# amazon-science/tubelet-transformer

Measured on AMD Instinct MI355X. Metric: clips/sec (TubeR CSN-152 AVA2.1 training step fwd+bwd+clip+AdamW, 32x256x340 clips; whole job), higher is better.
Workload: dtype bf16; 1 GPU; TubeR_CSN152_AVA21 train step, 2 clips/GPU of 3x32x256x340, dropout on, random-init name-hashed weights; global_batch=2, parallelism=dp1, launch_mode=hipgraph, lib_md5=41483701da62

## Files before the change

### include/tuber_hip.h

```cpp
#ifndef TUBER_HIP_H
#define TUBER_HIP_H

#ifdef __cplusplus
extern "C" {
#endif

typedef struct ihipStream_t* hipStream_t;

typedef struct TuberClipDesc {
    long long src_off;
    int H, W;
    int y1, x1, h, w;
    int flip, jitter;
    int hue, sat, val;
    int pad_;
} TuberClipDesc;

int tuber_attn_fwd(const void* Q, const long* mq, const void* K, const long* mk, const void* V, const long* mv, void* O, const long* mo, float* lse, const void* key_padding_mask, int B, int H, int Lq, int Lk, float scale, float pdrop, const void* seed_ptr, unsigned long long salt, hipStream_t stream);

int tuber_attn_bwd(const void* Q, const long* mq, const void* K, const long* mk, const void* V, const long* mv, const void* O, const long* mo, const float* lse, const void* key_padding_mask, const void* dO, const long* mdo, void* dQ, const long* mdq, void* dK, const long* mdk, void* dV, const long* mdv, float* delta, int B, int H, int Lq, int Lk, float scale, float pdrop, const void* seed_ptr, unsigned long long salt, hipStream_t stream);

int tuber_attn_wide_fwd(const void* q, const void* kv, void* o, int NQ, int HW, int T, float pdrop, const void* seed_ptr, unsigned long long salt, hipStream_t stream);

int tuber_attn_wide_bwd(const void* q, const void* kv, const void* dO, void* dq, void* dkv, int NQ, int HW, int T, float pdrop, const void* seed_ptr, unsigned long long salt, hipStream_t stream);

int tuber_blockout_conv1_supported(int c, int pn);

int tuber_blockout_conv1_fwd(const void* c4, const float* s4, const float* h4, const void* res, const float* rs, const float* rh, void* y, const void* w, long ldw, void* c1, float* st0, float* st1, long M, int pn, hipStream_t stream);

int tuber_blockout_conv1_fwd_mask(const void* c4, const float* s4, const float* h4, const void* res, const float* rs, const float* rh, void* y, void* ymask, const void* w, long ldw, void* c1, float* st0, float* st1, long M, int pn, hipStream_t stream);

int tuber_frames_resize(const void* src, void* tmp, void* dst, int nimg, int H, int W, int Ho, int Wo, const void* bounds_h, const void* kk_h, int ksize_h, const void* bounds_v, const void* kk_v, int ksize_v, int y0, int rows, hipStream_t stream);

int tuber_clip_prepare(const void* frames, const void* desc, const void* lut, const void* hsv_tab, void* out, void* mask, int N, int T, int Hmax, int Wmax, hipStream_t stream);

int tuber_clip_desc_bytes(void);

int tuber_comm_etimedout(void);

int tuber_comm_version(void);

const char* tuber_comm_last_error(void);

int tuber_comm_unique_id(void* id128);

int tuber_comm_init(const void* id128, int nranks, int rank, int device, void** comm_out);

int tuber_comm_init_timeout(const void* id128, int nranks, int rank, int device, int timeout_ms, void** comm_out);
// ... 273 lines not shown
```

### tubelet_transformer_amd/csrc/gen_header.py

```python
import glob
import os
import re

HERE = os.path.dirname(os.path.abspath(__file__))
ROOT = os.path.dirname(os.path.dirname(HERE))

DOC = {
    "tuber_gemm_nt_addproj": "packed attention in-projection with the positional embedding folded in: C = f(A).B^T + bias with f(A) = A + A2 for the output "
                             "columns [0, add_ncols) (q / k rows of in_proj_weight: with_pos_embed, models/transformer/transformer.py:150-159,215-240) and "
                             "f(A) = A for the v rows -- one GEMM instead of an add kernel and two GEMM launches. add_ncols % 128 == 0.",
    "tuber_bn_bwd_fa": "tuber_bn_bwd_finalize + tuber_bn_bwd_apply in ONE launch for short partial lists (layer3 / layer4 of the CSN body): every workgroup "
                       "derives the coefficients of its 128-channel strip from the R partial rows (fp64) and applies dx = cA*dz + cB*x + cC to its rows; "
                       "dgamma / dbeta accumulated by the first row chunk (NULL: frozen BatchNorm). autograd of nn.BatchNorm3d (ir_CSN_152.py:46,56,64,154).",
    "tuber_bn_bwd_fa_max_rows": "largest R tuber_bn_bwd_fa accepts.",
    "tuber_ln_bwd_dx": "tuber_layernorm_bwd (partial rows only) + the data-gradient tuber_gemm_nt of the linear layer in front of the LayerNorm in ONE launch: "
                       "autograd of tgt = norm(tgt + dropout(sublayer)) where the sublayer ends in out_proj / linear2 (models/transformer/transformer.py:160-167,229-247). "
                       "Every workgroup runs the LayerNorm backward of its 32 rows itself and multiplies the bf16 result from LDS with W on MFMA; the column-0 workgroups "
                       "store dx / dxd / the dgamma, dbeta partial rows ([tuber_ln_bwd_dx_blocks(M)][2E]) as the two-launch path does. dy2: a second gradient contribution (replaces "
                       "a tuber_axpby launch) or NULL; res: an existing gradient of the linear's input to add; cm / alpha: the ReLU / Dropout mask of that input.",
    "tuber_rows_dx2": "both data gradients of a packed attention in-projection with the positional embedding folded in (tuber_gemm_nt_addproj; "
                      "models/transformer/transformer.py:150-159,215-240) in ONE launch for few rows: dx = g.W over all N columns (+ res), dpos = g[:, :Nq].W[:Nq] "
                      "stored as a prefix of the same reduction. Replaces two tuber_gemm_nt launches per decoder in-projection.",
    "tuber_criterion_scale": "backward of tuber_criterion_loss's loss table in one launch: the stored per-layer gradients scaled by the incoming gradient of the [L][4] "
                             "losses (autograd of the weighted sum of loss terms, models/criterion.py:169-206 + train_tuber_ava.py loss weighting).",
# ... 210 lines not shown
    "tuber_block_out_bwd": "backward of the join: dz = dy*[y>0] and the partial statistics of bn4 (and of the down_sample BN).",
    "tuber_rowblock_count": "partial-stat rows written by the row-blocked reduce kernels for M rows.",
    "tuber_layernorm_fwd": "y = LayerNorm(Dropout_p(x) (+ res)) over E in {256, 2048}, eps 1e-5 (nn.LayerNorm, transformer.py:163-167,229-247,116-123; "
                           "transformer_layers.py:84,91,96,437-445); saves xhat (bf16) and rstd for backward.",
    "tuber_layernorm_bwd": "backward of tuber_layernorm_fwd: dx (gradient of res), dxd (gradient of x through the regenerated dropout mask) and dgamma/dbeta via block partials.",
    "tuber_layernorm_bwd_blocks": "blocks used by tuber_layernorm_bwd (partial = 2*blocks*E floats).",
    "tuber_reduce_rows": "out[c] (+)= sum_r P[r][c].",
    "tuber_colsum_blocks": "row blocks (size of `partial` / C) used by tuber_colsum.",
    "tuber_colsum": "bias gradient: out[c] (+)= sum_m g[m][c] for bf16 g.",
    "tuber_gemm_nt_set_cfg": "tuning hook: force tile configuration cfg for every later tuber_gemm_nt (-1 = automatic choice).",
    "tuber_stem_conv_fwd": "stem Conv3d(3,64,(3,7,7),s=(1,2,2),p=(1,3,3)) (ir_CSN_152.py:109-115) as an implicit MFMA GEMM from the fp32 NCDHW clip to NDHWC bf16, "
                           "with the partial statistics of the following BatchNorm; Wp = tuber_stem_pack_weight(conv1.weight).",
    "tuber_stem_conv_bwd_weight": "weight gradient of the stem conv ([64][441] fp32) as an implicit MFMA GEMM (no patch matrix in HBM).",
    "tuber_stem_conv_blocks": "persistent grid size of the stem conv forward = its partial-stat rows.",
    "tuber_stem_conv_wgrad_blocks": "workgroups (= [512][64] fp32 partial slabs) of tuber_stem_conv_bwd_weight.",
    "tuber_stem_pack_weight": "conv1.weight [64][441] fp32 -> [64][512] bf16 with k' = (c,kt,kh)*8 + kw (zero padded).",
    "tuber_stem_pool_fwd": "relu(bn1(.)) + MaxPool3d((1,3,3),s=(1,2,2),p=(0,1,1)) (ir_CSN_152.py:119-122) on NDHWC bf16, C=64; saves the argmax tap.",
    "tuber_stem_pool_bwd": "backward of the pool + relu(bn1(.)): dz and the BN-backward partial statistics.",
    "tuber_stem_pool_bwd_stat_rows": "partial-stat rows written by tuber_stem_pool_bwd.",
    "tuber_attn_fwd": "softmax(scale*QK^T + key_padding_mask)[dropout] V for 32-wide heads, operands read in place through strided token maps "
                      "{ld,sL,s1,s2,B2}: row(l,b) = l*sL + (b/B2)*s1 + (b%B2)*s2. Core of nn.MultiheadAttention "
                      "(transformer.py:159,227,237; tuber_ava.py:138; transformer_layers.py:81,88) and of the hand-rolled MHA (:156-167,306-366).",
    "tuber_attn_bwd": "gradients dQ, dK, dV of tuber_attn_fwd (P recomputed from the saved log-sum-exp).",
    "tuber_attn_wide_fwd": "single-query, 256-wide-head attention of the LSTR pooling decoder (TEMPORAL_DS_STRATEGY decode; "
                           "backbone_builder.py:74-78, transformer_layers.py:156-167,306-366): q [NQ,2048], kv [rows,4096]=[k|v], T<=8 slots per pixel.",
    "tuber_attn_wide_bwd": "gradients dq [NQ,2048] and dkv [rows,4096] of tuber_attn_wide_fwd.",
    "tuber_lsap": "rectangular linear sum assignment on HOST doubles; restates scipy.optimize.linear_sum_assignment (call sites "
                  "models/detr/matcher.py:80, matcher_ucf.py:82) incl. its tie-breaking.",
    "tuber_lsap_device": "the same assignment (scipy.optimize.linear_sum_assignment semantics incl. tie-breaking; matcher.py:80, matcher_ucf.py:82) for all "
                         "(decoder layer, clip) problems at once ON THE DEVICE, one thread per problem: match[l][b][t] = query of target t.",
    "tuber_grad_norm_clip_coef": "global L2 norm of the flat gradient buffer and the clip coefficient min(1, max_norm/(norm+1e-6)), left on the device: "
                                 "torch.nn.utils.clip_grad_norm_(model.parameters(), 0.1) (utils/video_action_recognition.py:153).  A non-finite norm "
                                 "yields coefficient -1 = skip the update and leaves the step count alone: the reference stops BEFORE optimizer.step() on a "
                                 "non-finite loss (video_action_recognition.py:195-198).",
    "tuber_adamw_segment": "AdamW update (torch.optim.AdamW semantics: decoupled decay, bias correction) of one contiguous flat segment with the "
                           "clip coefficient applied to the gradient on the fly (video_action_recognition.py:154; groups train_tuber_ava.py:41-58).",
    "tuber_grad_accum": "gradient accumulation over m micro-batches (DistributedDataParallel's mean over ranks reproduced on fewer GPUs: the mean of "
                        "independent per-rank backward passes, utils/model_utils.py:47-49) over a DEVICE table of nwin [begin, end) int64 windows of the flat "
                        "fp32 gradient buffer, in ONE launch: mode 0 acc = g, mode 1 acc += g, mode 2 g = (acc + g) * scale (scale_dev[0] when given). "
                        "Fixed order: sequential fp32 sum, then one multiply. g and acc 16-byte aligned.",
    "tuber_bn_stats_copy": "snapshot (restore = 0: arena <- buffers) or restore (restore = 1: buffers <- arena) of BatchNorm running statistics "
                           "(running_mean, running_var, num_batches_tracked of nn.BatchNorm3d, models/backbones/ir_CSN_152.py:46,56,64,154) in ONE launch over a "
                           "DEVICE table of nrows {address, arena offset in 32-bit words, words} int64 rows; max_words = the largest row.",
    "tuber_scale_f32": "x *= coef: gradient averaging after the RCCL all-reduce (DistributedDataParallel's mean, utils/model_utils.py:47-49).",
    "tuber_criterion_cost": "Hungarian matching cost C = w_bbox*L1 - w_giou*GIoU - w_class*p of every decoder layer at once, [L,B,Q,Tmax] fp32 "
                            "(HungarianMatcher.forward, models/detr/matcher.py:61-76 / matcher_ucf.py:61-78; generalized_box_iou utils/box_ops.py:41-65).",
# ... 101 lines not shown
```

### tubelet_transformer_amd/tape.py

```python
import numpy as np
import torch

from . import ab, lib

BF = torch.bfloat16


def _ceil(x, m):
    return (x + m - 1) // m * m


def _map(ld, sL, s1=0, s2=0, B2=1):
    return np.array([ld, sL, s1, s2, B2], dtype=np.int64)


class Tape:
    def __init__(self, store, train):
        self.store, self.train, self.dev = store, train, store.device
        self.ops = []
        self.g = {}
        self.alias = {}
        self.mask = {}
        self.premasked = set()
        self.stack = {}
# ... 407 lines not shown
            if acc == 2 and preq:
                if dbeta == dgamma + 4 * E:
                    st.defer.add(part, dgamma, 2 * E, 2 * E, nb, 1)
                else:
                    st.defer.add(part, dgamma, E, 2 * E, nb, 1)
                    st.defer.add(part + 4 * E, dbeta, E, 2 * E, nb, 1)
            return part, dgamma, dbeta, acc

        rec = _PendingLN(tp, g=g, gptr=gptr, ldg=ldg, g2=g2, xhat=xhat, rstd=rstd, gamma=gamma, dx=dx, dxd=dxd, p=p, salt=salt, M=M, E=E,
                         register=register)
        fusable = xreq and out is None and st.defer.enabled and not ab.on("no_ln_bwd_fusion") and id(tp.target(x)) in tp.lin_out
        chained = (xreq and out is not None and p == 0.0 and res is None and E == 256 and st.defer.enabled and not ab.on("no_ln_bwd_fusion")
                   and id(tp.target(x)) in tp.pair_ok and isinstance(tp.g.get(id(tp.target(x))), torch.Tensor))
        if not (fusable or chained):
            rec.force()
        if xreq:
            tp.put(x, dxd if p > 0.0 else dx)
        if rreq:
            tp.put(res, dx)
    tp.rec(bwd)
    return y


def attention(tp, roles, geom, kpm, pdrop, *tensors):
    st = tp.store
    B, H, Lq, Lk, qmap, kmap = geom
    (qi, qo), (ki, ko), (vi, vo) = roles
    tq, tk, tv = tensors[qi], tensors[ki], tensors[vi]
    dev = tq.device
    E = H * 32
    o = torch.empty(tq.shape[0], E, dtype=BF, device=dev)
    lse = torch.empty(B, H, Lq, dtype=torch.float32, device=dev)
    mq, mk, mv = _map(tq.shape[1], *qmap), _map(tk.shape[1], *kmap), _map(tv.shape[1], *kmap)
    mo = _map(E, *qmap)
    scale = 32 ** -0.5
    p = float(pdrop)
    salt = tp.salt()
    if tp.dry:
        tp.dry_log.append(("attention", dict(tensors=tensors, roles=roles, o=o, lse=lse, kpm=kpm, geom=geom, p=p, salt=salt)))
    else:
        lib.call("tuber_attn_fwd", tq.data_ptr() + 2 * qo, mq.ctypes.data, tk.data_ptr() + 2 * ko, mk.ctypes.data,
                 tv.data_ptr() + 2 * vo, mv.ctypes.data, o, mo.ctypes.data, lse, kpm, B, H, Lq, Lk, scale, float(p), st.seed, salt)
    if not tp.train:
        return o
    treq = [tp.needs(t) for t in tensors]
    if not any(treq):
        return o
    tp.mark(o)

    def bwd():
        g = tp.take(o)
        if g is None:
            return
        covered = [0] * len(tensors)
        for ti, _ in roles:
            covered[ti] += E
        grads = [torch.empty_like(t) if covered[i] >= t.shape[1] else torch.zeros_like(t) for i, t in enumerate(tensors)]
        delta = torch.empty(B, H, Lq, dtype=torch.float32, device=dev)
        lib.call("tuber_attn_bwd", tq.data_ptr() + 2 * qo, mq.ctypes.data, tk.data_ptr() + 2 * ko, mk.ctypes.data,
                 tv.data_ptr() + 2 * vo, mv.ctypes.data, o, mo.ctypes.data, lse, kpm, g, mo.ctypes.data,
                 grads[qi].data_ptr() + 2 * qo, mq.ctypes.data, grads[ki].data_ptr() + 2 * ko, mk.ctypes.data,
                 grads[vi].data_ptr() + 2 * vo, mv.ctypes.data, delta, B, H, Lq, Lk, scale, float(p), st.seed, salt)
        for t, gt, need in zip(tensors, grads, treq):
            if need:
                tp.put(t, gt)
    tp.rec(bwd)
    return o


def attention_wide(tp, q, kv, HW, T, pdrop):
    st = tp.store
    NQ = q.shape[0]
    o = torch.empty(NQ, 2048, dtype=BF, device=q.device)
    p = float(pdrop)
    salt = tp.salt()
    lib.call("tuber_attn_wide_fwd", q, kv, o, NQ, HW, T, float(p), st.seed, salt)
    if not tp.train:
        return o
    qreq, kreq = tp.needs(q), tp.needs(kv)
    if not (qreq or kreq):
        return o
    tp.mark(o)

    def bwd():
        g = tp.take(o)
# ... 175 lines not shown
```

### tubelet_transformer_amd/tuber.py

```python
import copy

import torch
from torch import nn

from . import ab, lib
from . import tape as T
from .backbone import build_CSN, CSNRunner
from .engine import ParamStore
from .misc import NestedTensor, nested_tensor_from_tensor_list

BF = torch.bfloat16


def _clones(m, n):
    return nn.ModuleList([copy.deepcopy(m) for _ in range(n)])


class TransformerEncoderLayer(nn.Module):
    def __init__(self, d_model, nhead, dim_feedforward, dropout):
        super().__init__()
        self.self_attn = nn.MultiheadAttention(d_model, nhead, dropout=dropout)
        self.linear1 = nn.Linear(d_model, dim_feedforward)
        self.dropout = nn.Dropout(dropout)
        self.linear2 = nn.Linear(dim_feedforward, d_model)
# ... 439 lines not shown
            x1, x2, boxes = (torch.empty(Rh, E, dtype=F32, device=dev), torch.empty(Rh, E, dtype=F32, device=dev), torch.empty(Rh, 4, dtype=F32, device=dev))
            lib.call("tuber_linear_f32", hs32, E, None, 0, 0, fp("bbox_embed.layers.0.weight"), E, fp("bbox_embed.layers.0.bias"), x1, E, Rh, E, E, 1)
            lib.call("tuber_linear_f32", x1, E, None, 0, 0, fp("bbox_embed.layers.1.weight"), E, fp("bbox_embed.layers.1.bias"), x2, E, Rh, E, E, 1)
            lib.call("tuber_linear_f32", x2, E, None, 0, 0, fp("bbox_embed.layers.2.weight"), E, fp("bbox_embed.layers.2.bias"), boxes, 4, Rh, 4, E, 2)
        else:
            x = T.linear(tp, hs, "bbox_embed.layers.0.weight", "bbox_embed.layers.0.bias", relu=True)
            x = T.linear(tp, x, "bbox_embed.layers.1.weight", "bbox_embed.layers.1.bias", relu=True)
            boxes = T.sigmoid(tp, T.linear(tp, x, "bbox_embed.layers.2.weight", "bbox_embed.layers.2.bias", out_f32=True))

        feat32, runner.last_y32 = runner.last_y32, None
        if hs32 is not None and ab.eval_class_f32():
            if feat32 is None:
                raise RuntimeError("TUBER_EVAL_PRECISION=fp32_class: the backbone did not produce its fp32 output stream")
            logits = self._class_branch_f32(st, feat32, hs32, B, Tp, hw, Q, lay_n, E, H)
        else:
            src_c = T.linear(tp, feat, "class_proj.weight", "class_proj.bias")
            R0 = B * Tp * hw
            rep = T.gather_sum(tp, src_c, (lay_n, 1, R0, 1, 0, 0, 1, 0, 1.0), (1, 1, R0, lay_n, 0, 0, 1, R0, 1.0))
            LB = lay_n * B
            cl = self.encoder.layers[0]
            pa_c, p1_c, pf_c = cl.self_attn_t.dropout * on, cl.dropout1.p * on, cl.dropout.p * on
            P = "encoder.layers.0"
            cat = torch.empty(lay_n * R0, 2 * E, dtype=BF, device=dev)
            qkv = T.linear(tp, rep, P + ".self_attn_t.in_proj_weight", P + ".self_attn_t.in_proj_bias")
            mp = (1, hw, 0, 1)
            a = T.attention(tp, ((0, 0), (0, E), (0, 2 * E)), (LB * Tp, H, hw, hw, mp, mp), None, pa_c, qkv)
            a = T.linear(tp, a, P + ".self_attn_t.out_proj.weight", P + ".self_attn_t.out_proj.bias")
            T.layer_norm(tp, a, rep, P + ".norm1_t", drop=p1_c, out=(cat, 0, 0))
            qkv = T.linear(tp, rep, P + ".self_attn_s.in_proj_weight", P + ".self_attn_s.in_proj_bias")
            mp = (hw, Tp * hw, 1, hw)
            a = T.attention(tp, ((0, 0), (0, E), (0, 2 * E)), (LB * hw, H, Tp, Tp, mp, mp), None, cl.self_attn_s.dropout * on, qkv)
            a = T.linear(tp, a, P + ".self_attn_s.out_proj.weight", P + ".self_attn_s.out_proj.bias")
            T.layer_norm(tp, a, rep, P + ".norm1_s", drop=p1_c, out=(cat, 0, E))
            enc = T.layer_norm(tp, self._ffn(tp, cat, P, pf_c), rep, P + ".norm2", drop=pf_c)
            q = T.linear(tp, hs, "cross_attn.in_proj_weight", "cross_attn.in_proj_bias", rows=(0, E))
            kv = T.linear(tp, enc, "cross_attn.in_proj_weight", "cross_attn.in_proj_bias", rows=(E, 3 * E))
            a = T.attention(tp, ((0, 0), (1, 0), (1, E)), (LB, H, Q, Tp * hw, (1, Q, 0, 1), (1, Tp * hw, 0, 1)), None,
                            self.cross_attn.dropout * on, q, kv)
            q_class = T.linear(tp, a, "cross_attn.out_proj.weight", "cross_attn.out_proj.bias", drop=self.dropout.p * on)
            logits = T.linear(tp, q_class, "class_fc.weight", "class_fc.bias", out_f32=True)
        shapes = ((lay_n, B, Q, logits.shape[1]), lb_shape, (lay_n, B, Q, 4))
        return tp, (logits, logits_b, boxes), shapes

    def _lstr_pool(self, tp, feat, B, Tp, hw, on):
        E = 2048
        P = "backbone.pool_decoder.layers.0"
        NQ = B * hw
        lay = self.backbone.pool_decoder.layers[0]
        p = lay.self_attn.dropout * on
        pr = lay.dropout1.p * on
        tgt = T.param_rows(tp, "backbone.query_pool.weight", NQ)
        S = P + ".self_attn"
        q = T.linear(tp, tgt, S + ".in_proj_weight", S + ".in_proj_bias", rows=(0, E))
        kv = T.linear(tp, tgt, S + ".in_proj_weight", S + ".in_proj_bias", rows=(E, 3 * E))
# ... 56 lines not shown
```

Measured before the change: 146.7 clips/s.

## Share replicated class-branch attention operands across layer copies instead of repeating them

```diff
diff --git a/include/tuber_hip.h b/include/tuber_hip.h
--- a/include/tuber_hip.h
+++ b/include/tuber_hip.h
@@ -24,6 +24,12 @@
 
 int tuber_attn_wide_bwd(const void* q, const void* kv, const void* dO, void* dq, void* dkv, int NQ, int HW, int T, float pdrop, const void* seed_ptr, unsigned long long salt, hipStream_t stream);
 
+int tuber_attn_shared_supported(int H, int Lq, int Lk, int copies);
+
+int tuber_attn_shared_fwd(const void* Q, const long* mq, const void* K, const long* mk, const void* V, const long* mv, void* O, const long* mo, float* lse, int B0, int H, int Lq, int Lk, int copies, float scale, float pdrop, const void* seed_ptr, unsigned long long salt, hipStream_t stream);
+
+int tuber_attn_shared_bwd(const void* Q, const long* mq, const void* K, const long* mk, const void* V, const long* mv, const void* O, const long* mo, const float* lse, const void* dO, const long* mdo, void* dQ, const long* mdq, void* dK, const long* mdk, void* dV, const long* mdv, float* delta, int B0, int H, int Lq, int Lk, int copies, float scale, float pdrop, const void* seed_ptr, unsigned long long salt, hipStream_t stream);
+
 int tuber_blockout_conv1_supported(int c, int pn);
 
 int tuber_blockout_conv1_fwd(const void* c4, const float* s4, const float* h4, const void* res, const float* rs, const float* rh, void* y, const void* w, long ldw, void* c1, float* st0, float* st1, long M, int pn, hipStream_t stream);
diff --git a/tubelet_transformer_amd/csrc/attention_shared.hip b/tubelet_transformer_amd/csrc/attention_shared.hip
--- /dev/null
+++ b/tubelet_transformer_amd/csrc/attention_shared.hip
@@ -0,0 +1,552 @@
+#include "attention.h"
+
+#include "attention_mfma_fwd.h"
+
+namespace {
+
+constexpr int NCOPY = 6;
+constexpr int FWD_NC = 3;
+constexpr int SMALL = 8;
+constexpr int SMALL_COPIES = 16;
+
+__device__ __forceinline__ uint64_t copy_stride(const AttnArgs& a) { return (uint64_t)a.B * a.H * a.Lq * (uint64_t)a.Lk; }
+
+template <int NC>
+__global__ __launch_bounds__(256) void attn_shared_fwd_kernel(AttnArgs a, int copies, int ntiles) {
+    __shared__ __attribute__((aligned(16))) bf16 ks[TL][RP];
+    __shared__ __attribute__((aligned(16))) bf16 vs[TL][RP];
+    const int cg = NC > 1 ? (int)blockIdx.x / ntiles * NC : 0;
+    const int b = blockIdx.z, h = blockIdx.y, q0 = ((int)blockIdx.x - (NC > 1 ? cg / NC * ntiles : 0)) * 64;
+    const int wave = threadIdx.x >> 6, lane = threadIdx.x & 63, li = lane & 15, g = lane >> 4;
+    const int qi = q0 + wave * 16 + li;
+    const bool qok = qi < a.Lq;
+    const int qc = qok ? qi : a.Lq - 1;
+    const bf16x8 qf = as_bf16x8(*(const uint4*)(a.Q + trow(a.mq, qc, b) * a.mq.ld + h * 32 + g * 8));
+    const float inv_keep = dropout_inv_keep(a.pdrop);
+    const uint64_t seed = a.pdrop > 0.f ? eseed(a.seed_ptr, a.salt) : 0ull;
+    const uint64_t cstride = copy_stride(a), rbase = cg * cstride + ((uint64_t)(b * a.H + h) * a.Lq + qc) * (uint64_t)a.Lk;
+    f32x4 o0[NC], o1[NC];
+#pragma unroll
+    for (int c = 0; c < NC; ++c) { o0[c] = f32x4{0.f, 0.f, 0.f, 0.f}; o1[c] = f32x4{0.f, 0.f, 0.f, 0.f}; }
+    float mx = -INFINITY, l = 0.f;
+    uint4 kr = tile_fetch(a.K, a.mk, b, h, 0, a.Lk), vr = tile_fetch(a.V, a.mv, b, h, 0, a.Lk);
+    for (int k0 = 0; k0 < a.Lk; k0 += TL) {
+        __syncthreads();
+        park_rm(ks, kr);
+        park_rm(vs, vr);
+        if (k0 + TL < a.Lk) { kr = tile_fetch(a.K, a.mk, b, h, k0 + TL, a.Lk); vr = tile_fetch(a.V, a.mv, b, h, k0 + TL, a.Lk); }
+        __syncthreads();
+#pragma unroll
+        for (int sub = 0; sub < 2; ++sub) {
+            const int c0 = sub * 32;
+            f32x4 s[2];
+#pragma unroll
+            for (int t = 0; t < 2; ++t) s[t] = mfma(frag_rm(ks, c0 + t * 16, li, g), qf, f32x4{0.f, 0.f, 0.f, 0.f});
+            float p[8];
+            float cmax = -INFINITY;
+#pragma unroll
+            for (int t = 0; t < 2; ++t)
+#pragma unroll
+                for (int r = 0; r < 4; ++r) {
+                    const bool dead = k0 + c0 + t * 16 + g * 4 + r >= a.Lk;
+                    p[t * 4 + r] = dead ? -INFINITY : s[t][r] * a.scale;
+                    cmax = fmaxf(cmax, p[t * 4 + r]);
+                }
+            cmax = group_max(cmax);
+            const float mnew = fmaxf(mx, cmax);
+            const float alpha = mnew == -INFINITY ? 1.f : __expf(mx - mnew);
+            float ls = 0.f;
+            bf16x8 pf0;
+            bool keep[2][4] = {{true, true, true, true}, {true, true, true, true}};
+            if (a.pdrop > 0.f) {
+                dropout_keep_run<4>(seed, rbase + k0 + c0 + g * 4, a.thresh, keep[0]);
+                dropout_keep_run<4>(seed, rbase + k0 + c0 + 16 + g * 4, a.thresh, keep[1]);
+            }
+#pragma unroll
+            for (int e = 0; e < 8; ++e) {
+                float pe = mnew == -INFINITY ? 0.f : __expf(p[e] - mnew);
+                ls += pe;
+                p[e] = pe;
+                if (a.pdrop > 0.f) pe = keep[e >> 2][e & 3] ? pe * inv_keep : 0.f;
+                pf0[e] = f2bf(pe);
+            }
+            l = l * alpha + group_sum(ls);
+            mx = mnew;
+            const bf16x8 v0 = frag_tr_rm(vs, 0, c0, li, g), v1 = frag_tr_rm(vs, 16, c0, li, g);
+#pragma unroll
+            for (int c = 0; c < NC; ++c) {
+                bf16x8 pf = pf0;
+                if (c > 0) {
+                    dropout_keep_run<4>(seed, c * cstride + rbase + k0 + c0 + g * 4, a.thresh, keep[0]);
+                    dropout_keep_run<4>(seed, c * cstride + rbase + k0 + c0 + 16 + g * 4, a.thresh, keep[1]);
+#pragma unroll
+                    for (int e = 0; e < 8; ++e) pf[e] = f2bf(keep[e >> 2][e & 3] ? p[e] * inv_keep : 0.f);
+                }
+#pragma unroll
+                for (int r = 0; r < 4; ++r) { o0[c][r] *= alpha; o1[c][r] *= alpha; }
+                o0[c] = mfma(v0, pf, o0[c]);
+                o1[c] = mfma(v1, pf, o1[c]);
+            }
+        }
+    }
+    if (qok) {
+        const float inv = l > 0.f ? 1.f / l : 0.f;
+        bf16x4 y0[NC], y1[NC];
+#pragma unroll
+        for (int c = 0; c < NC; ++c)
+#pragma unroll
+            for (int r = 0; r < 4; ++r) { y0[c][r] = f2bf(o0[c][r] * inv); y1[c][r] = f2bf(o1[c][r] * inv); }
+        if (NC > 1) {
+#pragma unroll
+            for (int c = 0; c < NC; ++c) {
+                bf16* orow = a.O + trow(a.mo, qi, (cg + c) * a.B + b) * a.mo.ld + h * 32;
+                *(uint2*)(orow + g * 4) = as_uint2(y0[c]);
+                *(uint2*)(orow + 16 + g * 4) = as_uint2(y1[c]);
+            }
+        } else {
+            for (int c = 0; c < copies; ++c) {
+                bf16* orow = a.O + trow(a.mo, qi, c * a.B + b) * a.mo.ld + h * 32;
+                *(uint2*)(orow + g * 4) = as_uint2(y0[0]);
+                *(uint2*)(orow + 16 + g * 4) = as_uint2(y1[0]);
+            }
+        }
+        if (g == 0 && cg == 0) a.lse[((long)b * a.H + h) * a.Lq + qi] = mx + __logf(l);
+    }
+}
+
+__global__ __launch_bounds__(256) void attn_shared_delta_kernel(AttnArgs a) {
+    const int bc = blockIdx.z, h = blockIdx.y;
+    const int lane = threadIdx.x & 63, li = lane & 15, g = lane >> 4;
+    const int qi = blockIdx.x * 64 + (threadIdx.x >> 6) * 16 + li;
+    const int qc = qi < a.Lq ? qi : a.Lq - 1;
+    const bf16x8 dof = as_bf16x8(*(const uint4*)(a.dO + trow(a.mdo, qc, bc) * a.mdo.ld + h * 32 + g * 8));
+    const bf16x8 of = as_bf16x8(*(const uint4*)(a.O + trow(a.mo, qc, bc) * a.mo.ld + h * 32 + g * 8));
+    float d = 0.f;
+#pragma unroll
+    for (int e = 0; e < 8; ++e) d = fmaf(bf2f(dof[e]), bf2f(of[e]), d);
+    d = group_sum(d);
+    if (qi < a.Lq && g == 0) a.delta[((long)bc * a.H + h) * a.Lq + qi] = d;
+}
+
+constexpr int DQ_LDS = 2 * TL * RP * (int)sizeof(bf16);
+constexpr int DKV_LDS = (1 + NCOPY) * TL * RP * (int)sizeof(bf16) + (1 + NCOPY) * TL * (int)sizeof(float);
+
+__device__ __forceinline__ void attn_shared_bwd_dq_body(const AttnArgs& a, const int bx, char* sm) {
+    constexpr int NC = NCOPY;
+    bf16 (*ks)[RP] = (bf16 (*)[RP])sm;
+    bf16 (*vs)[RP] = (bf16 (*)[RP])(sm + TL * RP * sizeof(bf16));
+    const int b = blockIdx.z, h = blockIdx.y, q0 = bx * 64;
+    const int wave = threadIdx.x >> 6, lane = threadIdx.x & 63, li = lane & 15, g = lane >> 4;
+    const int qi = q0 + wave * 16 + li;
+    const bool qok = qi < a.Lq;
+    const int qc = qok ? qi : a.Lq - 1;
+    const bf16x8 qf = as_bf16x8(*(const uint4*)(a.Q + trow(a.mq, qc, b) * a.mq.ld + h * 32 + g * 8));
+    const long dstride = (long)a.B * a.H * a.Lq;
+    bf16x8 dof[NC];
+    float delta[NC];
+#pragma unroll
+    for (int c = 0; c < NC; ++c) {
+        dof[c] = as_bf16x8(*(const uint4*)(a.dO + trow(a.mdo, qc, c * a.B + b) * a.mdo.ld + h * 32 + g * 8));
+        delta[c] = a.delta[c * dstride + ((long)b * a.H + h) * a.Lq + qc];
+    }
+    const float lse = a.lse[((long)b * a.H + h) * a.Lq + qc];
+    const float inv_keep = dropout_inv_keep(a.pdrop);
+    const uint64_t seed = a.pdrop > 0.f ? eseed(a.seed_ptr, a.salt) : 0ull;
+    const uint64_t rbase = ((uint64_t)(b * a.H + h) * a.Lq + qc) * (uint64_t)a.Lk, cstride = copy_stride(a);
+    f32x4 dq0 = {0.f, 0.f, 0.f, 0.f}, dq1 = {0.f, 0.f, 0.f, 0.f};
+    uint4 kr = tile_fetch(a.K, a.mk, b, h, 0, a.Lk), vr = tile_fetch(a.V, a.mv, b, h, 0, a.Lk);
+    for (int k0 = 0; k0 < a.Lk; k0 += TL) {
+        __syncthreads();
+        park_rm(ks, kr);
+        park_rm(vs, vr);
+        if (k0 + TL < a.Lk) { kr = tile_fetch(a.K, a.mk, b, h, k0 + TL, a.Lk); vr = tile_fetch(a.V, a.mv, b, h, k0 + TL, a.Lk); }
+        __syncthreads();
+#pragma unroll
+        for (int sub = 0; sub < 2; ++sub) {
+            const int c0 = sub * 32;
+            float p[8];
+            bf16x8 vf[2];
+#pragma unroll
+            for (int t = 0; t < 2; ++t) {
+                const f32x4 s = mfma(frag_rm(ks, c0 + t * 16, li, g), qf, f32x4{0.f, 0.f, 0.f, 0.f});
+                vf[t] = frag_rm(vs, c0 + t * 16, li, g);
+#pragma unroll
+                for (int r = 0; r < 4; ++r) p[t * 4 + r] = k0 + c0 + t * 16 + g * 4 + r >= a.Lk ? 0.f : __expf(s[r] * a.scale - lse);
+            }
+            const bf16x8 kt0 = frag_tr_rm(ks, 0, c0, li, g), kt1 = frag_tr_rm(ks, 16, c0, li, g);
+#pragma unroll
+            for (int c = 0; c < NC; ++c) {
+                bf16x8 dsf;
+#pragma unroll
+                for (int t = 0; t < 2; ++t) {
+                    const f32x4 dp = mfma(vf[t], dof[c], f32x4{0.f, 0.f, 0.f, 0.f});
+                    bool keep[4] = {true, true, true, true};
+                    if (a.pdrop > 0.f) dropout_keep_run<4>(seed, c * cstride + rbase + k0 + c0 + t * 16 + g * 4, a.thresh, keep);
+#pragma unroll
+                    for (int r = 0; r < 4; ++r) {
+                        float dpv = dp[r];
+                        if (a.pdrop > 0.f) dpv = keep[r] ? dpv * inv_keep : 0.f;
+                        dsf[t * 4 + r] = f2bf(p[t * 4 + r] * (dpv - delta[c]) * a.scale);
+                    }
+                }
+                dq0 = mfma(kt0, dsf, dq0);
+                dq1 = mfma(kt1, dsf, dq1);
+            }
+        }
+    }
+    if (qok) {
+        bf16* orow = a.dQ + trow(a.mdq, qi, b) * a.mdq.ld + h * 32;
+        bf16x4 y0, y1;
+#pragma unroll
+        for (int r = 0; r < 4; ++r) { y0[r] = f2bf(dq0[r]); y1[r] = f2bf(dq1[r]); }
+        *(uint2*)(orow + g * 4) = as_uint2(y0);
+        *(uint2*)(orow + 16 + g * 4) = as_uint2(y1);
+    }
+}
+
+__device__ __forceinline__ void attn_shared_bwd_dkv_body(const AttnArgs& a, const int bx, char* sm) {
+    constexpr int NC = NCOPY;
+    bf16 (*qs)[RP] = (bf16 (*)[RP])sm;
+    bf16 (*dos)[TL][RP] = (bf16 (*)[TL][RP])(sm + TL * RP * sizeof(bf16));
+    float* lse_s = (float*)(sm + (1 + NC) * TL * RP * sizeof(bf16));
+    float (*del_s)[TL] = (float (*)[TL])(sm + (1 + NC) * TL * RP * sizeof(bf16) + TL * sizeof(float));
+    const int b = blockIdx.z, h = blockIdx.y, kb = bx * 64;
+    const int wave = threadIdx.x >> 6, lane = threadIdx.x & 63, li = lane & 15, g = lane >> 4;
+    const int ki = kb + wave * 16 + li;
+    const bool kin = ki < a.Lk;
+    const int kc = kin ? ki : a.Lk - 1;
+    const bf16x8 kf = as_bf16x8(*(const uint4*)(a.K + trow(a.mk, kc, b) * a.mk.ld + h * 32 + g * 8));
+    const bf16x8 vf = as_bf16x8(*(const uint4*)(a.V + trow(a.mv, kc, b) * a.mv.ld + h * 32 + g * 8));
+    const float inv_keep = dropout_inv_keep(a.pdrop);
+    const uint64_t seed = a.pdrop > 0.f ? eseed(a.seed_ptr, a.salt) : 0ull;
+    const uint64_t bh = (uint64_t)(b * a.H + h), cstride = copy_stride(a);
+    const long dstride = (long)a.B * a.H * a.Lq;
+    const bool pair_words = (a.Lk & 1) == 0;
+    f32x4 dk0 = {0.f, 0.f, 0.f, 0.f}, dk1 = {0.f, 0.f, 0.f, 0.f}, dv0 = {0.f, 0.f, 0.f, 0.f}, dv1 = {0.f, 0.f, 0.f, 0.f};
+    const int srow = (int)threadIdx.x;
+    uint4 qr = tile_fetch(a.Q, a.mq, b, h, 0, a.Lq), dr[NC];
+    float lr = 0.f, er[NC];
+#pragma unroll
+    for (int c = 0; c < NC; ++c) {
+        dr[c] = tile_fetch(a.dO, a.mdo, c * a.B + b, h, 0, a.Lq);
+        er[c] = 0.f;
+    }
+    if (srow < TL && srow < a.Lq) {
+        lr = a.lse[bh * a.Lq + srow];
+#pragma unroll
+        for (int c = 0; c < NC; ++c) er[c] = a.delta[c * dstride + bh * a.Lq + srow];
+    }
+    for (int q0 = 0; q0 < a.Lq; q0 += TL) {
+        __syncthreads();
+        park_rm(qs, qr);
+#pragma unroll
+        for (int c = 0; c < NC; ++c) park_rm(dos[c], dr[c]);
+        if (srow < TL) {
+            lse_s[srow] = lr;
+#pragma unroll
+            for (int c = 0; c < NC; ++c) del_s[c][srow] = er[c];
+        }
+        if (q0 + TL < a.Lq) {
+            qr = tile_fetch(a.Q, a.mq, b, h, q0 + TL, a.Lq);
+#pragma unroll
+            for (int c = 0; c < NC; ++c) dr[c] = tile_fetch(a.dO, a.mdo, c * a.B + b, h, q0 + TL, a.Lq);
+            const int qn = q0 + TL + srow;
+            if (srow < TL) {
+                const bool in = qn < a.Lq;
+                lr = in ? a.lse[bh * a.Lq + qn] : 0.f;
+#pragma unroll
+                for (int c = 0; c < NC; ++c) er[c] = in ? a.delta[c * dstride + bh * a.Lq + qn] : 0.f;
+            }
+        }
+        __syncthreads();
+#pragma unroll
+        for (int sub = 0; sub < 2; ++sub) {
+            const int c0 = sub * 32;
+            float p[8];
+#pragma unroll
+            for (int t = 0; t < 2; ++t) {
+                const f32x4 s = mfma(frag_rm(qs, c0 + t * 16, li, g), kf, f32x4{0.f, 0.f, 0.f, 0.f});
+#pragma unroll
+                for (int r = 0; r < 4; ++r) {
+                    const int ql = c0 + t * 16 + g * 4 + r;
+                    p[t * 4 + r] = (kin && q0 + ql < a.Lq) ? __expf(s[r] * a.scale - lse_s[ql]) : 0.f;
+                }
+            }
+            const bf16x8 qt0 = frag_tr_rm(qs, 0, c0, li, g), qt1 = frag_tr_rm(qs, 16, c0, li, g);
+#pragma unroll
+            for (int c = 0; c < NC; ++c) {
+                bf16x8 pf, dsf;
+                uint32_t wd[2][4];
+                if (a.pdrop > 0.f) {
+                    const uint64_t kbase = c * cstride + bh * a.Lq * (uint64_t)a.Lk + kc;
+                    if (pair_words) {
+                        const int tm = li & 1;
+                        uint32_t mine[4], other[4];
+#pragma unroll
+                        for (int r = 0; r < 4; ++r) {
+                            mine[r] = dropout_word(seed, (kbase + (uint64_t)(q0 + c0 + tm * 16 + g * 4 + r) * a.Lk) >> 1);
+                            other[r] = __builtin_amdgcn_update_dpp(0, mine[r], DPP_XOR1, 0xF, 0xF, true);
+                        }
+#pragma unroll
+                        for (int r = 0; r < 4; ++r) { wd[0][r] = tm ? other[r] : mine[r]; wd[1][r] = tm ? mine[r] : other[r]; }
+                    } else {
+#pragma unroll
+                        for (int t = 0; t < 2; ++t)
+#pragma unroll
+                            for (int r = 0; r < 4; ++r) wd[t][r] = dropout_word(seed, (kbase + (uint64_t)(q0 + c0 + t * 16 + g * 4 + r) * a.Lk) >> 1);
+                    }
+                }
+#pragma unroll
+                for (int t = 0; t < 2; ++t) {
+                    const f32x4 dp = mfma(frag_rm(dos[c], c0 + t * 16, li, g), vf, f32x4{0.f, 0.f, 0.f, 0.f});
+#pragma unroll
+                    for (int r = 0; r < 4; ++r) {
+                        const int ql = c0 + t * 16 + g * 4 + r;
+                        const float pe = p[t * 4 + r];
+                        float pd = pe, dpv = dp[r];
+                        if (a.pdrop > 0.f) {
+                            const uint64_t idx = c * cstride + (bh * a.Lq + (uint64_t)(q0 + ql)) * (uint64_t)a.Lk + kc;
+                            const bool keep = ((idx & 1) ? (wd[t][r] >> 16) : (wd[t][r] & 0xFFFFu)) >= (a.thresh >> 16);
+                            pd = keep ? pe * inv_keep : 0.f;
+                            dpv = keep ? dpv * inv_keep : 0.f;
+                        }
+                        pf[t * 4 + r] = f2bf(pd);
+                        dsf[t * 4 + r] = f2bf(pe * (dpv - del_s[c][ql]) * a.scale);
+                    }
+                }
+                dv0 = mfma(frag_tr_rm(dos[c], 0, c0, li, g), pf, dv0);
+                dv1 = mfma(frag_tr_rm(dos[c], 16, c0, li, g), pf, dv1);
+                dk0 = mfma(qt0, dsf, dk0);
+                dk1 = mfma(qt1, dsf, dk1);
+            }
+        }
+    }
+    if (kin) {
+        bf16* krow = a.dK + trow(a.mdk, ki, b) * a.mdk.ld + h * 32;
+        bf16* vrow = a.dV + trow(a.mdv, ki, b) * a.mdv.ld + h * 32;
+        bf16x4 y0, y1, z0, z1;
+#pragma unroll
+        for (int r = 0; r < 4; ++r) { y0[r] = f2bf(dk0[r]); y1[r] = f2bf(dk1[r]); z0[r] = f2bf(dv0[r]); z1[r] = f2bf(dv1[r]); }
+        *(uint2*)(krow + g * 4) = as_uint2(y0);
+        *(uint2*)(krow + 16 + g * 4) = as_uint2(y1);
+        *(uint2*)(vrow + g * 4) = as_uint2(z0);
+        *(uint2*)(vrow + 16 + g * 4) = as_uint2(z1);
+    }
+}
+
+__global__ __launch_bounds__(256, 3) void attn_shared_bwd_kernel(AttnArgs a, int nq) {
+    __shared__ __attribute__((aligned(16))) char sm[DKV_LDS > DQ_LDS ? DKV_LDS : DQ_LDS];
+    if ((int)blockIdx.x < nq) attn_shared_bwd_dq_body(a, blockIdx.x, sm);
+    else attn_shared_bwd_dkv_body(a, (int)blockIdx.x - nq, sm);
+}
+
+__device__ __forceinline__ void ld32(const bf16* p, float (&v)[32]) {
+#pragma unroll
+    for (int i = 0; i < 4; ++i) {
+        const bf16x8 t = as_bf16x8(((const uint4*)p)[i]);
+#pragma unroll
+        for (int e = 0; e < 8; ++e) v[i * 8 + e] = bf2f(t[e]);
+    }
+}
+__device__ __forceinline__ void st32(bf16* p, const float (&v)[32]) {
+#pragma unroll
+    for (int i = 0; i < 4; ++i) {
+        bf16x8 t;
+#pragma unroll
+        for (int e = 0; e < 8; ++e) t[e] = f2bf(v[i * 8 + e]);
+        ((uint4*)p)[i] = as_uint4(t);
+    }
+}
+__device__ __forceinline__ float dot32s(const float (&a)[32], const float (&b)[32]) {
+    float s0 = 0.f, s1 = 0.f, s2 = 0.f, s3 = 0.f;
+#pragma unroll
+    for (int d = 0; d < 32; d += 4) {
+        s0 = fmaf(a[d], b[d], s0); s1 = fmaf(a[d + 1], b[d + 1], s1);
+        s2 = fmaf(a[d + 2], b[d + 2], s2); s3 = fmaf(a[d + 3], b[d + 3], s3);
+    }
+    return (s0 + s1) + (s2 + s3);
+}
+
+__global__ __launch_bounds__(64) void attn_shared_small_fwd_kernel(AttnArgs a, int copies) {
+    const long t = (long)blockIdx.x * 64 + threadIdx.x;
+    if (t >= (long)a.B * a.H * a.Lq) return;
+    const int h = (int)(t % a.H), qi = (int)((t / a.H) % a.Lq), b = (int)(t / ((long)a.H * a.Lq));
+    const long li = ((long)b * a.H + h) * a.Lq + qi;
+    float q[32], o[32], p[SMALL];
+    ld32(a.Q + trow(a.mq, qi, b) * a.mq.ld + h * 32, q);
+    float mx = -INFINITY;
+#pragma unroll
+    for (int k = 0; k < SMALL; ++k) {
+        p[k] = -INFINITY;
+        if (k < a.Lk) {
+            float kv[32];
+            ld32(a.K + trow(a.mk, k, b) * a.mk.ld + h * 32, kv);
+            p[k] = dot32s(q, kv) * a.scale;
+            mx = fmaxf(mx, p[k]);
+        }
+    }
+    float l = 0.f;
+#pragma unroll
+    for (int k = 0; k < SMALL; ++k)
+        if (k < a.Lk) { p[k] = __expf(p[k] - mx); l += p[k]; }
+    const float inv = l > 0.f ? 1.f / l : 0.f;
+    const float inv_keep = dropout_inv_keep(a.pdrop);
+    const uint64_t seed = a.pdrop > 0.f ? eseed(a.seed_ptr, a.salt) : 0ull;
+    const uint64_t cstride = copy_stride(a);
+    for (int c = 0; c < copies; ++c) {
+        if (c == 0 || a.pdrop > 0.f) {
+#pragma unroll
+            for (int d = 0; d < 32; ++d) o[d] = 0.f;
+#pragma unroll
+            for (int k = 0; k < SMALL; ++k) {
+                if (k < a.Lk) {
+                    float pv = p[k];
+                    if (a.pdrop > 0.f) pv = dropout_keep(seed, c * cstride + (uint64_t)li * a.Lk + k, a.thresh) ? p[k] * inv_keep : 0.f;
+                    float vv[32];
+                    ld32(a.V + trow(a.mv, k, b) * a.mv.ld + h * 32, vv);
+#pragma unroll
+                    for (int d = 0; d < 32; ++d) o[d] = fmaf(pv, vv[d], o[d]);
+                }
+            }
+#pragma unroll
+            for (int d = 0; d < 32; ++d) o[d] *= inv;
+        }
+        st32(a.O + trow(a.mo, qi, c * a.B + b) * a.mo.ld + h * 32, o);
+    }
+    a.lse[li] = mx + __logf(l);
+}
+
+__global__ __launch_bounds__(64) void attn_shared_small_bwd_kernel(AttnArgs a, int copies) {
+    const bool keys = blockIdx.y == 1;
+    const int L = keys ? a.Lk : a.Lq;
+    const long t = (long)blockIdx.x * 64 + threadIdx.x;
+    if (t >= (long)a.B * a.H * L) return;
+    const int h = (int)(t % a.H), i = (int)((t / a.H) % L), b = (int)(t / ((long)a.H * L));
+    const long bh = (long)b * a.H + h;
+    const long dstride = (long)a.B * a.H * a.Lq;
+    const float inv_keep = dropout_inv_keep(a.pdrop);
+    const uint64_t seed = a.pdrop > 0.f ? eseed(a.seed_ptr, a.salt) : 0ull;
+    const uint64_t cstride = copy_stride(a);
+    if (!keys) {
+        float q[32], dq[32], p[SMALL];
+        ld32(a.Q + trow(a.mq, i, b) * a.mq.ld + h * 32, q);
+        const long li = bh * a.Lq + i;
+        const float lse = a.lse[li];
+#pragma unroll
+        for (int k = 0; k < SMALL; ++k) {
+            p[k] = 0.f;
+            if (k < a.Lk) {
+                float kv[32];
+                ld32(a.K + trow(a.mk, k, b) * a.mk.ld + h * 32, kv);
+                p[k] = __expf(dot32s(q, kv) * a.scale - lse);
+            }
+        }
+#pragma unroll
+        for (int d = 0; d < 32; ++d) dq[d] = 0.f;
+        for (int c = 0; c < copies; ++c) {
+            const int bc = c * a.B + b;
+            float dov[32], ov[32];
+            ld32(a.dO + trow(a.mdo, i, bc) * a.mdo.ld + h * 32, dov);
+            ld32(a.O + trow(a.mo, i, bc) * a.mo.ld + h * 32, ov);
+            const float delta = dot32s(dov, ov);
+            a.delta[c * dstride + li] = delta;
+#pragma unroll
+            for (int k = 0; k < SMALL; ++k) {
+                if (k < a.Lk) {
+                    float kv[32], vv[32];
+                    ld32(a.K + trow(a.mk, k, b) * a.mk.ld + h * 32, kv);
+                    ld32(a.V + trow(a.mv, k, b) * a.mv.ld + h * 32, vv);
+                    float dp = dot32s(dov, vv);
+                    if (a.pdrop > 0.f) dp = dropout_keep(seed, c * cstride + (uint64_t)li * a.Lk + k, a.thresh) ? dp * inv_keep : 0.f;
+                    const float ds = p[k] * (dp - delta) * a.scale;
+#pragma unroll
+                    for (int d = 0; d < 32; ++d) dq[d] = fmaf(ds, kv[d], dq[d]);
+                }
+            }
+        }
+        st32(a.dQ + trow(a.mdq, i, b) * a.mdq.ld + h * 32, dq);
+    } else {
+        float k[32], v[32], dk[32], dv[32];
+        ld32(a.K + trow(a.mk, i, b) * a.mk.ld + h * 32, k);
+        ld32(a.V + trow(a.mv, i, b) * a.mv.ld + h * 32, v);
+#pragma unroll
+        for (int d = 0; d < 32; ++d) { dk[d] = 0.f; dv[d] = 0.f; }
+        for (int qq = 0; qq < a.Lq; ++qq) {
+            float qv[32];
+            ld32(a.Q + trow(a.mq, qq, b) * a.mq.ld + h * 32, qv);
+            const long li = bh * a.Lq + qq;
+            const float p = __expf(dot32s(qv, k) * a.scale - a.lse[li]);
+            for (int c = 0; c < copies; ++c) {
+                const int bc = c * a.B + b;
+                float dov[32], ov[32];
+                ld32(a.dO + trow(a.mdo, qq, bc) * a.mdo.ld + h * 32, dov);
+                ld32(a.O + trow(a.mo, qq, bc) * a.mo.ld + h * 32, ov);
+                float dp = dot32s(dov, v), pd = p;
+                if (a.pdrop > 0.f) {
+                    const bool keep = dropout_keep(seed, c * cstride + (uint64_t)li * a.Lk + i, a.thresh);
+                    pd = keep ? p * inv_keep : 0.f;
+                    dp = keep ? dp * inv_keep : 0.f;
+                }
+                const float ds = p * (dp - dot32s(dov, ov)) * a.scale;
+#pragma unroll
+                for (int d = 0; d < 32; ++d) { dv[d] = fmaf(pd, dov[d], dv[d]); dk[d] = fmaf(ds, qv[d], dk[d]); }
+            }
+        }
+        st32(a.dK + trow(a.mdk, i, b) * a.mdk.ld + h * 32, dk);
+        st32(a.dV + trow(a.mdv, i, b) * a.mdv.ld + h * 32, dv);
+    }
+}
+
+TokMap mk_map(const long* m) { TokMap t; t.ld = m[0]; t.sL = m[1]; t.s1 = m[2]; t.s2 = m[3]; t.B2 = (int)m[4]; return t; }
+
+}
+
+extern "C" {
+
+int tuber_attn_shared_supported(int H, int Lq, int Lk, int copies) {
+    if (H <= 0 || Lq <= 0 || Lk <= 0 || copies < 1) return 0;
+    if (Lq <= SMALL && Lk <= SMALL) return copies <= SMALL_COPIES ? 1 : 0;
+    return copies == NCOPY ? 1 : 0;
+}
+
+int tuber_attn_shared_fwd(const void* Q, const long* mq, const void* K, const long* mk, const void* V, const long* mv, void* O,
+                          const long* mo, float* lse, int B0, int H, int Lq, int Lk, int copies, float scale, float pdrop,
+                          const void* seed_ptr, unsigned long long salt, hipStream_t stream) {
+    if (B0 <= 0 || pdrop < 0.f || pdrop >= 1.f || !lse || !tuber_attn_shared_supported(H, Lq, Lk, copies)) return TUBER_EINVAL;
+    AttnArgs a{};
+    a.Q = (const bf16*)Q; a.mq = mk_map(mq); a.K = (const bf16*)K; a.mk = mk_map(mk); a.V = (const bf16*)V; a.mv = mk_map(mv);
+    a.O = (bf16*)O; a.mo = mk_map(mo); a.lse = lse;
+    a.B = B0; a.H = H; a.Lq = Lq; a.Lk = Lk; a.scale = scale; a.pdrop = pdrop;
+    a.thresh = (uint32_t)((double)pdrop * 4294967296.0); a.seed_ptr = (const uint64_t*)seed_ptr; a.salt = salt;
+    if (Lq <= SMALL && Lk <= SMALL)
+        hipLaunchKernelGGL(attn_shared_small_fwd_kernel, dim3(ceil_div((long)B0 * H * Lq, 64)), dim3(64), 0, stream, a, copies);
+    else if (pdrop > 0.f)
+        hipLaunchKernelGGL(attn_shared_fwd_kernel<FWD_NC>, dim3(ceil_div(Lq, 64) * (NCOPY / FWD_NC), H, B0), dim3(256), 0, stream, a, copies, ceil_div(Lq, 64));
+    else
+        hipLaunchKernelGGL(attn_shared_fwd_kernel<1>, dim3(ceil_div(Lq, 64), H, B0), dim3(256), 0, stream, a, copies, ceil_div(Lq, 64));
+    TUBER_RETURN_LAUNCH();
+}
+
+int tuber_attn_shared_bwd(const void* Q, const long* mq, const void* K, const long* mk, const void* V, const long* mv, const void* O,
+                          const long* mo, const float* lse, const void* dO, const long* mdo, void* dQ, const long* mdq, void* dK,
+                          const long* mdk, void* dV, const long* mdv, float* delta, int B0, int H, int Lq, int Lk, int copies, float scale,
+                          float pdrop, const void* seed_ptr, unsigned long long salt, hipStream_t stream) {
+    if (B0 <= 0 || pdrop < 0.f || pdrop >= 1.f || !lse || !delta || !tuber_attn_shared_supported(H, Lq, Lk, copies)) return TUBER_EINVAL;
+    AttnArgs a{};
+    a.Q = (const bf16*)Q; a.mq = mk_map(mq); a.K = (const bf16*)K; a.mk = mk_map(mk); a.V = (const bf16*)V; a.mv = mk_map(mv);
+    a.O = (bf16*)O; a.mo = mk_map(mo); a.lse = (float*)lse;
+    a.B = B0; a.H = H; a.Lq = Lq; a.Lk = Lk; a.scale = scale; a.pdrop = pdrop;
+    a.thresh = (uint32_t)((double)pdrop * 4294967296.0); a.seed_ptr = (const uint64_t*)seed_ptr; a.salt = salt;
+    a.dO = (const bf16*)dO; a.mdo = mk_map(mdo); a.dQ = (bf16*)dQ; a.mdq = mk_map(mdq); a.dK = (bf16*)dK; a.mdk = mk_map(mdk);
+    a.dV = (bf16*)dV; a.mdv = mk_map(mdv); a.delta = delta;
+    if (Lq <= SMALL && Lk <= SMALL) {
+        hipLaunchKernelGGL(attn_shared_small_bwd_kernel, dim3(ceil_div((long)B0 * H * (Lq > Lk ? Lq : Lk), 64), 2), dim3(64), 0, stream, a, copies);
+    } else {
+        const int nq = ceil_div(Lq, 64), nk = ceil_div(Lk, 64);
+        hipLaunchKernelGGL(attn_shared_delta_kernel, dim3(nq, H, copies * B0), dim3(256), 0, stream, a);
+        hipLaunchKernelGGL(attn_shared_bwd_kernel, dim3(nq + nk, H, B0), dim3(256), 0, stream, a, nq);
+    }
+    TUBER_RETURN_LAUNCH();
+}
+
+}
diff --git a/tubelet_transformer_amd/csrc/gen_header.py b/tubelet_transformer_amd/csrc/gen_header.py
--- a/tubelet_transformer_amd/csrc/gen_header.py
+++ b/tubelet_transformer_amd/csrc/gen_header.py
@@ -256,6 +256,18 @@
                       "{ld,sL,s1,s2,B2}: row(l,b) = l*sL + (b/B2)*s1 + (b%B2)*s2. Core of nn.MultiheadAttention "
                       "(transformer.py:159,227,237; tuber_ava.py:138; transformer_layers.py:81,88) and of the hand-rolled MHA (:156-167,306-366).",
     "tuber_attn_bwd": "gradients dQ, dK, dV of tuber_attn_fwd (P recomputed from the saved log-sum-exp).",
+    "tuber_attn_shared_fwd": "tuber_attn_fwd on an operand replicated `copies` times, without the replicas: Q / K / V hold B0 batch entries, O holds copies * B0 "
+                             "(batch index c * B0 + b through the same token map), lse is [B0][H][Lq]. The class branch runs one encoder layer on src_c repeated "
+                             "lay_n times (models/tuber_ava.py:129-135) and nothing in front of self_attn_t / self_attn_s makes the copies differ "
+                             "(transformer_layers.py:79-91: no dropout, no positional term), so scores, row maximum, exp and lse are formed once; copy c then applies "
+                             "the dropout mask tuber_attn_fwd draws for batch index c * B0 + b and accumulates its own P_c V: every copy's O is bit-identical to "
+                             "tuber_attn_fwd on the replicated operand (64-row form). pdrop == 0: computed once, stored copies times. No key-padding mask.",
+    "tuber_attn_shared_bwd": "gradients of tuber_attn_shared_fwd: dO and delta hold copies * B0 batch entries, dQ / dK / dV B0 -- the sum over the copies "
+                             "(autograd of the repeat in models/tuber_ava.py:133 followed by nn.MultiheadAttention, transformer_layers.py:79-91). P_c and dS_c are "
+                             "rounded to bf16 per copy as in tuber_attn_bwd and accumulated in ONE fp32 accumulator over the copies; one rounding at the store.",
+    "tuber_attn_shared_supported": "1 when tuber_attn_shared_fwd / _bwd take (H, Lq, Lk, copies): Lq, Lk <= 8 (self_attn_s over the temporal slots, transformer_layers.py:86-91) with up "
+                                   "to 16 copies, or the MFMA kernels (self_attn_t, transformer_layers.py:79-84) with exactly 6 copies (lay_n of models/tuber_ava.py:129-135); 0: the caller "
+                                   "replicates and runs tuber_attn_fwd / tuber_attn_bwd.",
     "tuber_attn_wide_fwd": "single-query, 256-wide-head attention of the LSTR pooling decoder (TEMPORAL_DS_STRATEGY decode; "
                            "backbone_builder.py:74-78, transformer_layers.py:156-167,306-366): q [NQ,2048], kv [rows,4096]=[k|v], T<=8 slots per pixel.",
     "tuber_attn_wide_bwd": "gradients dq [NQ,2048] and dkv [rows,4096] of tuber_attn_wide_fwd.",
diff --git a/tubelet_transformer_amd/tape.py b/tubelet_transformer_amd/tape.py
--- a/tubelet_transformer_amd/tape.py
+++ b/tubelet_transformer_amd/tape.py
@@ -1,3 +1,5 @@
+import os
+
 import numpy as np
 import torch
 
@@ -453,14 +455,20 @@
     return y
 
 
-def attention(tp, roles, geom, kpm, pdrop, *tensors):
+def class_shared():
+    return os.environ.get("TUBER_CLASS_SHARED", "1") != "0"
+
+
+def attention(tp, roles, geom, kpm, pdrop, *tensors, copies=1):
     st = tp.store
     B, H, Lq, Lk, qmap, kmap = geom
     (qi, qo), (ki, ko), (vi, vo) = roles
     tq, tk, tv = tensors[qi], tensors[ki], tensors[vi]
     dev = tq.device
     E = H * 32
-    o = torch.empty(tq.shape[0], E, dtype=BF, device=dev)
+    if copies > 1 and (kpm is not None or tp.dry):
+        raise ValueError("attention(copies=%d): no key-padding mask and no dry run on the shared-operand path" % copies)
+    o = torch.empty(copies * tq.shape[0], E, dtype=BF, device=dev)
     lse = torch.empty(B, H, Lq, dtype=torch.float32, device=dev)
     mq, mk, mv = _map(tq.shape[1], *qmap), _map(tk.shape[1], *kmap), _map(tv.shape[1], *kmap)
     mo = _map(E, *qmap)
@@ -469,6 +477,9 @@
     salt = tp.salt()
     if tp.dry:
         tp.dry_log.append(("attention", dict(tensors=tensors, roles=roles, o=o, lse=lse, kpm=kpm, geom=geom, p=p, salt=salt)))
+    elif copies > 1:
+        lib.call("tuber_attn_shared_fwd", tq.data_ptr() + 2 * qo, mq.ctypes.data, tk.data_ptr() + 2 * ko, mk.ctypes.data,
+                 tv.data_ptr() + 2 * vo, mv.ctypes.data, o, mo.ctypes.data, lse, B, H, Lq, Lk, copies, scale, float(p), st.seed, salt)
     else:
         lib.call("tuber_attn_fwd", tq.data_ptr() + 2 * qo, mq.ctypes.data, tk.data_ptr() + 2 * ko, mk.ctypes.data,
                  tv.data_ptr() + 2 * vo, mv.ctypes.data, o, mo.ctypes.data, lse, kpm, B, H, Lq, Lk, scale, float(p), st.seed, salt)
@@ -487,11 +498,17 @@
         for ti, _ in roles:
             covered[ti] += E
         grads = [torch.empty_like(t) if covered[i] >= t.shape[1] else torch.zeros_like(t) for i, t in enumerate(tensors)]
-        delta = torch.empty(B, H, Lq, dtype=torch.float32, device=dev)
-        lib.call("tuber_attn_bwd", tq.data_ptr() + 2 * qo, mq.ctypes.data, tk.data_ptr() + 2 * ko, mk.ctypes.data,
-                 tv.data_ptr() + 2 * vo, mv.ctypes.data, o, mo.ctypes.data, lse, kpm, g, mo.ctypes.data,
-                 grads[qi].data_ptr() + 2 * qo, mq.ctypes.data, grads[ki].data_ptr() + 2 * ko, mk.ctypes.data,
-                 grads[vi].data_ptr() + 2 * vo, mv.ctypes.data, delta, B, H, Lq, Lk, scale, float(p), st.seed, salt)
+        delta = torch.empty(copies * B, H, Lq, dtype=torch.float32, device=dev)
+        if copies > 1:
+            lib.call("tuber_attn_shared_bwd", tq.data_ptr() + 2 * qo, mq.ctypes.data, tk.data_ptr() + 2 * ko, mk.ctypes.data,
+                     tv.data_ptr() + 2 * vo, mv.ctypes.data, o, mo.ctypes.data, lse, g, mo.ctypes.data,
+                     grads[qi].data_ptr() + 2 * qo, mq.ctypes.data, grads[ki].data_ptr() + 2 * ko, mk.ctypes.data,
+                     grads[vi].data_ptr() + 2 * vo, mv.ctypes.data, delta, B, H, Lq, Lk, copies, scale, float(p), st.seed, salt)
+        else:
+            lib.call("tuber_attn_bwd", tq.data_ptr() + 2 * qo, mq.ctypes.data, tk.data_ptr() + 2 * ko, mk.ctypes.data,
+                     tv.data_ptr() + 2 * vo, mv.ctypes.data, o, mo.ctypes.data, lse, kpm, g, mo.ctypes.data,
+                     grads[qi].data_ptr() + 2 * qo, mq.ctypes.data, grads[ki].data_ptr() + 2 * ko, mk.ctypes.data,
+                     grads[vi].data_ptr() + 2 * vo, mv.ctypes.data, delta, B, H, Lq, Lk, scale, float(p), st.seed, salt)
         for t, gt, need in zip(tensors, grads, treq):
             if need:
                 tp.put(t, gt)
diff --git a/tubelet_transformer_amd/tuber.py b/tubelet_transformer_amd/tuber.py
--- a/tubelet_transformer_amd/tuber.py
+++ b/tubelet_transformer_amd/tuber.py
@@ -485,14 +485,18 @@
             pa_c, p1_c, pf_c = cl.self_attn_t.dropout * on, cl.dropout1.p * on, cl.dropout.p * on
             P = "encoder.layers.0"
             cat = torch.empty(lay_n * R0, 2 * E, dtype=BF, device=dev)
-            qkv = T.linear(tp, rep, P + ".self_attn_t.in_proj_weight", P + ".self_attn_t.in_proj_bias")
+            sh_t = T.class_shared() and lib.query("tuber_attn_shared_supported", H, hw, hw, lay_n) == 1
+            sh_s = T.class_shared() and lib.query("tuber_attn_shared_supported", H, Tp, Tp, lay_n) == 1
+            qkv = T.linear(tp, src_c if sh_t else rep, P + ".self_attn_t.in_proj_weight", P + ".self_attn_t.in_proj_bias")
             mp = (1, hw, 0, 1)
-            a = T.attention(tp, ((0, 0), (0, E), (0, 2 * E)), (LB * Tp, H, hw, hw, mp, mp), None, pa_c, qkv)
+            a = T.attention(tp, ((0, 0), (0, E), (0, 2 * E)), ((B if sh_t else LB) * Tp, H, hw, hw, mp, mp), None, pa_c, qkv,
+                            copies=lay_n if sh_t else 1)
             a = T.linear(tp, a, P + ".self_attn_t.out_proj.weight", P + ".self_attn_t.out_proj.bias")
             T.layer_norm(tp, a, rep, P + ".norm1_t", drop=p1_c, out=(cat, 0, 0))
-            qkv = T.linear(tp, rep, P + ".self_attn_s.in_proj_weight", P + ".self_attn_s.in_proj_bias")
+            qkv = T.linear(tp, src_c if sh_s else rep, P + ".self_attn_s.in_proj_weight", P + ".self_attn_s.in_proj_bias")
             mp = (hw, Tp * hw, 1, hw)
-            a = T.attention(tp, ((0, 0), (0, E), (0, 2 * E)), (LB * hw, H, Tp, Tp, mp, mp), None, cl.self_attn_s.dropout * on, qkv)
+            a = T.attention(tp, ((0, 0), (0, E), (0, 2 * E)), ((B if sh_s else LB) * hw, H, Tp, Tp, mp, mp), None, cl.self_attn_s.dropout * on, qkv,
+                            copies=lay_n if sh_s else 1)
             a = T.linear(tp, a, P + ".self_attn_s.out_proj.weight", P + ".self_attn_s.out_proj.bias")
             T.layer_norm(tp, a, rep, P + ".norm1_s", drop=p1_c, out=(cat, 0, E))
             enc = T.layer_norm(tp, self._ffn(tp, cat, P, pf_c), rep, P + ".norm2", drop=pf_c)
```

Result: no change. 147.9 clips/s, median of 6 (+0.8%).
